# martenlienen/bsi

Hardware: AMD Instinct MI355X
Metric: images/sec BSI.sample k=128 (DiT, 3x32x32) (higher is better)
Workload: dtype bf16

## Files before the change

### bsi_amd/csrc/dit_ops.hip

```cpp
#include <math.h>

#include "common.h"
#include "dit_ops.h"

namespace {

constexpr int TPB = 256;

__global__ void silu_bf16_kernel(const float* __restrict__ pre, size_t n, __bf16* __restrict__ out) {
    for (size_t i = (size_t)blockIdx.x * blockDim.x + threadIdx.x; i < n; i += (size_t)gridDim.x * blockDim.x)
        out[i] = (__bf16)silu_f(pre[i]);
}

__global__ void cast_bf16_kernel(const float* __restrict__ in, int ld_in, int rows, int cols, __bf16* __restrict__ out, int ld) {
    const int r = blockIdx.y;
    const float* ir = in + (size_t)r * ld_in;
    __bf16* orow = out + (size_t)r * ld;
    for (int c = (blockIdx.x * blockDim.x + threadIdx.x) * 4; c < ld; c += gridDim.x * blockDim.x * 4) {
        float v[4];
#pragma unroll
        for (int k = 0; k < 4; ++k) v[k] = (c + k < cols) ? ir[c + k] : 0.0f;
        if (c + 3 < ld) {
            u32x2 w;
            w[0] = pack_bf16x2(v[0], v[1]);
            w[1] = pack_bf16x2(v[2], v[3]);
            *reinterpret_cast<u32x2*>(orow + c) = w;
        } else {
            for (int k = 0; k < 4 && c + k < ld; ++k) orow[c + k] = (__bf16)v[k];
        }
    }
}

__global__ void nyquist_kernel(const float* __restrict__ t, int rows, const float* __restrict__ scale,
                               const float* __restrict__ bias, int size, float* __restrict__ of, __bf16* __restrict__ ob) {
    const int r = blockIdx.y;
    const float tv = t[r];
    for (int j = blockIdx.x * blockDim.x + threadIdx.x; j < size; j += gridDim.x * blockDim.x) {
        const float v = sinf(__fmaf_rn(scale[j], tv, bias[j]));
        if (of) of[(size_t)r * size + j] = v;
        if (ob) ob[(size_t)r * size + j] = (__bf16)v;
    }
}

template <int VPL, bool MASKGEN = false>
__global__ void ln_modulate_kernel(float* __restrict__ x, int M, int d, float eps, const float* __restrict__ shift,
                                   const float* __restrict__ scale, int mod_rows, int mod_stride, int tokens,
                                   const float* __restrict__ ln_w, const float* __restrict__ ln_b,
                                   const __bf16* delta, const float* __restrict__ gate, __bf16* out, DropCfg dc,
                                   float* x_out, float* __restrict__ stats, const __bf16* delta0 = nullptr,
                                   const float* __restrict__ gate0 = nullptr, int write_x = 1, DropCfg mdc = DropCfg{},
                                   unsigned long long* __restrict__ maskw = nullptr) {
    const int lane = threadIdx.x & 63;
    const int row = blockIdx.x * (blockDim.x >> 6) + (threadIdx.x >> 6);
    if (row >= M) return;
    if constexpr (MASKGEN) maskw[(size_t)row * 64 + lane] = drop_mask_block(mdc, (unsigned)row, lane);
    const float* xr = x + (size_t)row * d;
    float* xw = (x_out ? x_out : x) + (size_t)row * d;
    const int d4 = d >> 2;
    const int mrow = (shift || gate || gate0) ? (row / tokens) % mod_rows : 0;
    f32x4 v[VPL];
    float s = 0.f;
#pragma unroll
    for (int i = 0; i < VPL; ++i) {
        const int c = i * 64 + lane;
        v[i] = (c < d4) ? reinterpret_cast<const f32x4*>(xr)[c] : f32x4{0.f, 0.f, 0.f, 0.f};
        if (delta0 && c < d4) {
            const u32x2 dw = __builtin_nontemporal_load(reinterpret_cast<const u32x2*>(delta0 + (size_t)row * d) + c);
            const f32x4 g = reinterpret_cast<const f32x4*>(gate0 + (size_t)mrow * mod_stride)[c];
            v[i][0] = __fmaf_rn(g[0], __uint_as_float(dw[0] << 16), v[i][0]);
            v[i][1] = __fmaf_rn(g[1], __uint_as_float(dw[0] & 0xffff0000u), v[i][1]);
            v[i][2] = __fmaf_rn(g[2], __uint_as_float(dw[1] << 16), v[i][2]);
            v[i][3] = __fmaf_rn(g[3], __uint_as_float(dw[1] & 0xffff0000u), v[i][3]);
        }
        if (delta && c < d4) {
            const u32x2 dw = __builtin_nontemporal_load(reinterpret_cast<const u32x2*>(delta + (size_t)row * d) + c);
            const f32x4 g = reinterpret_cast<const f32x4*>(gate + (size_t)mrow * mod_stride)[c];
            v[i][0] = __fmaf_rn(g[0], __uint_as_float(dw[0] << 16), v[i][0]);
            v[i][1] = __fmaf_rn(g[1], __uint_as_float(dw[0] & 0xffff0000u), v[i][1]);
            v[i][2] = __fmaf_rn(g[2], __uint_as_float(dw[1] << 16), v[i][2]);
            v[i][3] = __fmaf_rn(g[3], __uint_as_float(dw[1] & 0xffff0000u), v[i][3]);
            if (write_x) reinterpret_cast<f32x4*>(xw)[c] = v[i];
        }
        s += (v[i][0] + v[i][1]) + (v[i][2] + v[i][3]);
    }
    if (!out) return;
    const float mean = wave_sum(s) / (float)d;
    float q = 0.f;
#pragma unroll
    for (int i = 0; i < VPL; ++i) {
        const int c = i * 64 + lane;
        if (c < d4) {
#pragma unroll
            for (int k = 0; k < 4; ++k) {
                const float dd = v[i][k] - mean;
                q = __fmaf_rn(dd, dd, q);
            }
        }
    }
    const float rstd = 1.0f / sqrtf(wave_sum(q) / (float)d + eps);
    if (stats && lane == 0) {
        stats[2 * (size_t)row] = mean;
        stats[2 * (size_t)row + 1] = rstd;
    }
    const float* sh = shift ? shift + (size_t)mrow * mod_stride : nullptr;
    const float* sc = scale ? scale + (size_t)mrow * mod_stride : nullptr;
    __bf16* orow = out + (size_t)row * d;
#pragma unroll
    for (int i = 0; i < VPL; ++i) {
        const int c = i * 64 + lane;
        if (c < d4) {
            f32x4 y;
#pragma unroll
            for (int k = 0; k < 4; ++k) y[k] = (v[i][k] - mean) * rstd;
            if (sh) {
                const f32x4 a = reinterpret_cast<const f32x4*>(sh)[c];
                const f32x4 b = reinterpret_cast<const f32x4*>(sc)[c];
#pragma unroll
                for (int k = 0; k < 4; ++k) y[k] = __fmaf_rn(b[k] + 1.0f, y[k], a[k]);
            } else if (ln_w) {
                const f32x4 a = reinterpret_cast<const f32x4*>(ln_w)[c];
                const f32x4 b = reinterpret_cast<const f32x4*>(ln_b)[c];
#pragma unroll
                for (int k = 0; k < 4; ++k) y[k] = __fmaf_rn(y[k], a[k], b[k]);
            }
            if (dc.thr) {
                const unsigned rh = drop_row(dc, (unsigned)row);
#pragma unroll
                for (int k = 0; k < 4; ++k) y[k] = drop_keep_rc(dc, rh, (unsigned)c * 4 + k) ? y[k] * dc.scale : 0.0f;
            }
            u32x2 w;
            w[0] = pack_bf16x2(y[0], y[1]);
            w[1] = pack_bf16x2(y[2], y[3]);
            reinterpret_cast<u32x2*>(orow)[c] = w;
        }
    }
}

template <int VPL>
__global__ __launch_bounds__(256) void ln_modulate_stream_kernel(float* __restrict__ x, int M, int d, float eps, const float* __restrict__ shift,
                                                                 const float* __restrict__ scale, const __bf16* delta0,
                                                                 const float* __restrict__ gate0, const __bf16* delta,
                                                                 const float* __restrict__ gate, int write_x, __bf16* out) {
    __shared__ f32x4 tab[4][VPL * 64];
    const int d4 = d >> 2;
    for (int i = threadIdx.x; i < VPL * 64; i += blockDim.x) {
        const f32x4 z{0.f, 0.f, 0.f, 0.f};
        const bool in = i < d4;
        tab[0][i] = (gate0 && in) ? reinterpret_cast<const f32x4*>(gate0)[i] : z;
        tab[1][i] = (gate && in) ? reinterpret_cast<const f32x4*>(gate)[i] : z;
        tab[2][i] = in ? reinterpret_cast<const f32x4*>(shift)[i] : z;
        tab[3][i] = in ? reinterpret_cast<const f32x4*>(scale)[i] : z;
    }
    __syncthreads();
    const int lane = threadIdx.x & 63;
    const int wpb = blockDim.x >> 6;
    const int stride = gridDim.x * wpb;
    int row = blockIdx.x * wpb + (threadIdx.x >> 6);
    const bool has0 = delta0 != nullptr, has1 = delta != nullptr;

    struct Row {
        f32x4 v[VPL];
        u32x2 a[VPL], b[VPL];
    };
    auto load = [&](int r, Row& R) {
        const float* xr = x + (size_t)r * d;
#pragma unroll
        for (int i = 0; i < VPL; ++i) {
            const int c = i * 64 + lane;
            R.v[i] = (c < d4) ? reinterpret_cast<const f32x4*>(xr)[c] : f32x4{0.f, 0.f, 0.f, 0.f};
            if (has0 && c < d4) R.a[i] = __builtin_nontemporal_load(reinterpret_cast<const u32x2*>(delta0 + (size_t)r * d) + c);
            if (has1 && c < d4) R.b[i] = __builtin_nontemporal_load(reinterpret_cast<const u32x2*>(delta + (size_t)r * d) + c);
        }
    };
    auto finish = [&](int r, Row& R) {
        float* xw = x + (size_t)r * d;
        float s = 0.f;
#pragma unroll
        for (int i = 0; i < VPL; ++i) {
            const int c = i * 64 + lane;
            if (has0 && c < d4) {
                const f32x4 g = tab[0][c];
                R.v[i][0] = __fmaf_rn(g[0], __uint_as_float(R.a[i][0] << 16), R.v[i][0]);
                R.v[i][1] = __fmaf_rn(g[1], __uint_as_float(R.a[i][0] & 0xffff0000u), R.v[i][1]);
                R.v[i][2] = __fmaf_rn(g[2], __uint_as_float(R.a[i][1] << 16), R.v[i][2]);
                R.v[i][3] = __fmaf_rn(g[3], __uint_as_float(R.a[i][1] & 0xffff0000u), R.v[i][3]);
            }
            if (has1 && c < d4) {
                const f32x4 g = tab[1][c];
                R.v[i][0] = __fmaf_rn(g[0], __uint_as_float(R.b[i][0] << 16), R.v[i][0]);
                R.v[i][1] = __fmaf_rn(g[1], __uint_as_float(R.b[i][0] & 0xffff0000u), R.v[i][1]);
                R.v[i][2] = __fmaf_rn(g[2], __uint_as_float(R.b[i][1] << 16), R.v[i][2]);
                R.v[i][3] = __fmaf_rn(g[3], __uint_as_float(R.b[i][1] & 0xffff0000u), R.v[i][3]);
                if (write_x) reinterpret_cast<f32x4*>(xw)[c] = R.v[i];
            }
            s += (R.v[i][0] + R.v[i][1]) + (R.v[i][2] + R.v[i][3]);
        }
        const float mean = wave_sum(s) / (float)d;
        float q = 0.f;
#pragma unroll
        for (int i = 0; i < VPL; ++i) {
            const int c = i * 64 + lane;
            if (c < d4) {
#pragma unroll
                for (int k = 0; k < 4; ++k) {
                    const float dd = R.v[i][k] - mean;
                    q = __fmaf_rn(dd, dd, q);
                }
            }
        }
        const float rstd = 1.0f / sqrtf(wave_sum(q) / (float)d + eps);
        __bf16* orow = out + (size_t)r * d;
#pragma unroll
        for (int i = 0; i < VPL; ++i) {
            const int c = i * 64 + lane;
            if (c < d4) {
                f32x4 y;
#pragma unroll
                for (int k = 0; k < 4; ++k) y[k] = (R.v[i][k] - mean) * rstd;
                const f32x4 a = tab[2][c];
                const f32x4 b = tab[3][c];
#pragma unroll
                for (int k = 0; k < 4; ++k) y[k] = __fmaf_rn(b[k] + 1.0f, y[k], a[k]);
                u32x2 w;
                w[0] = pack_bf16x2(y[0], y[1]);
                w[1] = pack_bf16x2(y[2], y[3]);
                reinterpret_cast<u32x2*>(orow)[c] = w;
            }
        }
    };
    Row A, B;
    if (row >= M) return;
    load(row, A);
    while (true) {
        if (row + stride < M) load(row + stride, B);
        finish(row, A);
        row += stride;
        if (row >= M) break;
        if (row + stride < M) load(row + stride, A);
        finish(row, B);
        row += stride;
        if (row >= M) break;
    }
}

__global__ void fourier_features_kernel(const float* __restrict__ x, size_t total, int C, int inner, int nmin,
                                        int nfreq, float* __restrict__ out) {
    for (size_t idx = (size_t)blockIdx.x * blockDim.x + threadIdx.x; idx < total; idx += (size_t)gridDim.x * blockDim.x) {
        const size_t in_i = idx % inner;
        const size_t oc = idx / inner;
        const float v = x[idx];
        float* o = out + (oc * nfreq * 2) * inner + in_i;
        for (int n = 0; n < nfreq; ++n) {
            const float coef = 6.283185307179586f * (float)(1 << (nmin + n));
            o[(size_t)(n * 2 + 0) * inner] = sinf(__fmaf_rn(coef, v, 0.0f));
            o[(size_t)(n * 2 + 1) * inner] = sinf(__fmaf_rn(coef, v, 1.5707963267948966f));
        }
    }
}

__global__ void dit_prologue_kernel(const float* __restrict__ mu, const float* __restrict__ c_in, int coef_stride, int B,
                                    int C, int H, int W, int ps, int nmin, int nfreq, int kpad, __bf16* __restrict__ out) {
    const int HW = H * W;
    const size_t total = (size_t)B * HW;
    const int Cin = C + C * nfreq * 2;
    const int nw = W / ps;
    const int tokens = (H / ps) * nw;
    const int K = ps * ps * Cin;
    for (size_t idx = (size_t)blockIdx.x * blockDim.x + threadIdx.x; idx < total; idx += (size_t)gridDim.x * blockDim.x) {
        const int b = (int)(idx / HW);
        const int pix = (int)(idx % HW);
        const int h = pix / W, w = pix % W;
        const float ci = c_in ? c_in[(size_t)b * coef_stride] : 1.0f;
        const int tok = (h / ps) * nw + (w / ps);
        const int intra = (h % ps) * ps + (w % ps);
        __bf16* o = out + ((size_t)b * tokens + tok) * kpad + intra * Cin;
        for (int c = 0; c < C; ++c) {
            float v = mu[((size_t)b * C + c) * HW + pix];
            if (c_in) v = __fmul_rn(ci, v);
            o[c] = (__bf16)v;
            for (int n = 0; n < nfreq; ++n) {
                const float coef = 6.283185307179586f * (float)(1 << (nmin + n));
                o[C + (c * nfreq + n) * 2 + 0] = (__bf16)sinf(__fmaf_rn(coef, v, 0.0f));
                o[C + (c * nfreq + n) * 2 + 1] = (__bf16)sinf(__fmaf_rn(coef, v, 1.5707963267948966f));
            }
        }
        if (intra == ps * ps - 1) {
            __bf16* z = out + ((size_t)b * tokens + tok) * kpad;
            for (int c = K; c < kpad; ++c) z[c] = (__bf16)0.0f;
        }
    }
}

template <int VPL, bool WLDS>
__global__ void dit_final_kernel(const float* __restrict__ x, int Mtok, int d, int P, const float* __restrict__ ln_w,
                                 const float* __restrict__ ln_b, const float* __restrict__ dec_w,
                                 const float* __restrict__ dec_b, int C, int H, int W, int ps,
                                 const float* __restrict__ mu, const float* __restrict__ c_skip,
                                 const float* __restrict__ c_out, int coef_stride, const __bf16* __restrict__ delta,
                                 const float* __restrict__ gate, int gate_rows, int gate_stride,
                                 float* __restrict__ out) {
    extern __shared__ __attribute__((aligned(16))) float wsm[];
    const int d4 = d >> 2;
    if constexpr (WLDS) {
        for (int i = threadIdx.x; i < P * d4; i += blockDim.x)
            reinterpret_cast<f32x4*>(wsm)[i] = reinterpret_cast<const f32x4*>(dec_w)[i];
        __syncthreads();
    }
    const int lane = threadIdx.x & 63;
    const int wpb = blockDim.x >> 6;
    const int nw = W / ps;
    const int tokens = (H / ps) * nw;
    const int HW = H * W;
    constexpr int FR = 4;
    for (int row0 = (blockIdx.x * wpb + (threadIdx.x >> 6)) * FR; row0 < Mtok; row0 += gridDim.x * wpb * FR) {
        f32x4 v[FR][VPL];
        float s[FR], q[FR];
#pragma unroll
        for (int r = 0; r < FR; ++r) {
            const int row = row0 + r < Mtok ? row0 + r : Mtok - 1;
            const float* xr = x + (size_t)row * d;
            const int b_idx = row / tokens;
            s[r] = 0.f;
#pragma unroll
            for (int i = 0; i < VPL; ++i) {
                const int c = i * 64 + lane;
                v[r][i] = (c < d4) ? reinterpret_cast<const f32x4*>(xr)[c] : f32x4{0.f, 0.f, 0.f, 0.f};
                if (delta && c < d4) {
                    const u32x2 dw = reinterpret_cast<const u32x2*>(delta + (size_t)row * d)[c];
                    const f32x4 g = reinterpret_cast<const f32x4*>(gate + (size_t)(b_idx % gate_rows) * gate_stride)[c];
                    v[r][i][0] = __fmaf_rn(g[0], __uint_as_float(dw[0] << 16), v[r][i][0]);
                    v[r][i][1] = __fmaf_rn(g[1], __uint_as_float(dw[0] & 0xffff0000u), v[r][i][1]);
                    v[r][i][2] = __fmaf_rn(g[2], __uint_as_float(dw[1] << 16), v[r][i][2]);
                    v[r][i][3] = __fmaf_rn(g[3], __uint_as_float(dw[1] & 0xffff0000u), v[r][i][3]);
                }
                s[r] += (v[r][i][0] + v[r][i][1]) + (v[r][i][2] + v[r][i][3]);
            }
        }
#pragma unroll
        for (int m = 32; m > 0; m >>= 1)
#pragma unroll
            for (int r = 0; r < FR; ++r) s[r] += __shfl_xor(s[r], m, 64);
#pragma unroll
        for (int r = 0; r < FR; ++r) {
            const float mean = s[r] / (float)d;
            s[r] = mean;
            q[r] = 0.f;
#pragma unroll
            for (int i = 0; i < VPL; ++i) {
                const int c = i * 64 + lane;
                if (c < d4) {
#pragma unroll
                    for (int k = 0; k < 4; ++k) {
                        const float dd = v[r][i][k] - mean;
                        q[r] = __fmaf_rn(dd, dd, q[r]);
                    }
                }
            }
        }
#pragma unroll
        for (int m = 32; m > 0; m >>= 1)
#pragma unroll
            for (int r = 0; r < FR; ++r) q[r] += __shfl_xor(q[r], m, 64);
#pragma unroll
        for (int i = 0; i < VPL; ++i) {
            const int c = i * 64 + lane;
            if (c < d4) {
                const f32x4 a = reinterpret_cast<const f32x4*>(ln_w)[c];
                const f32x4 bb = reinterpret_cast<const f32x4*>(ln_b)[c];
#pragma unroll
                for (int r = 0; r < FR; ++r) {
                    const float rstd = 1.0f / sqrtf(q[r] / (float)d + 1e-5f);
#pragma unroll
                    for (int k = 0; k < 4; ++k) v[r][i][k] = __fmaf_rn((v[r][i][k] - s[r]) * rstd, a[k], bb[k]);
                }
            }
        }
        float mine[FR] = {0.f, 0.f, 0.f, 0.f};
        for (int o0 = 0; o0 < P; o0 += 4) {
            float acc[FR][4];
#pragma unroll
            for (int r = 0; r < FR; ++r)
#pragma unroll
                for (int u = 0; u < 4; ++u) acc[r][u] = 0.f;
#pragma unroll
            for (int u = 0; u < 4; ++u) {
                const int o = o0 + u < P ? o0 + u : P - 1;
#pragma unroll
                for (int i = 0; i < VPL; ++i) {
                    const int c = i * 64 + lane;
                    if (c < d4) {
                        const f32x4 wv = WLDS ? reinterpret_cast<const f32x4*>(wsm + (size_t)o * d)[c]
                                              : reinterpret_cast<const f32x4*>(dec_w + (size_t)o * d)[c];
#pragma unroll
                        for (int r = 0; r < FR; ++r)
#pragma unroll
                            for (int k = 0; k < 4; ++k) acc[r][u] = __fmaf_rn(v[r][i][k], wv[k], acc[r][u]);
                    }
                }
            }
#pragma unroll
            for (int m = 32; m > 0; m >>= 1)
#pragma unroll
                for (int r = 0; r < FR; ++r)
#pragma unroll
                    for (int u = 0; u < 4; ++u) acc[r][u] += __shfl_xor(acc[r][u], m, 64);
#pragma unroll
            for (int u = 0; u < 4; ++u)
                if (o0 + u < P && lane == o0 + u) {
#pragma unroll
                    for (int r = 0; r < FR; ++r) mine[r] = acc[r][u] + dec_b[o0 + u];
                }
        }
        if (lane < P) {
            const int intra = lane / C, ch = lane % C;
#pragma unroll
            for (int r = 0; r < FR; ++r) {
                const int row = row0 + r;
                if (row >= Mtok) break;
                const int b_idx = row / tokens, tok = row % tokens;
                const int th = tok / nw, tw = tok % nw;
                const int hh = th * ps + intra / ps, ww = tw * ps + intra % ps;
                const size_t gi = ((size_t)b_idx * C + ch) * HW + (size_t)hh * W + ww;
                float rr = mine[r];
                if (c_skip) {
                    const float cs = c_skip[(size_t)b_idx * coef_stride], co = c_out[(size_t)b_idx * coef_stride];
                    rr = __fmaf_rn(co, mine[r], __fmul_rn(cs, mu[gi]));
                }
                out[gi] = rr;
            }
        }
    }
}

}

#define S(stream) reinterpret_cast<hipStream_t>(stream)

extern "C" int bsi_cast_rows_bf16(const float* in, int ld_in, int rows, int cols, void* out, int ld_out,
                                  bsi_stream_t stream) {
    BSI_CHECK_ARG(in && out && rows > 0 && cols > 0 && ld_in >= cols && ld_out >= cols && ld_out % 4 == 0,
                  "bsi_cast_rows_bf16: bad args rows=%d cols=%d ld_in=%d ld_out=%d", rows, cols, ld_in, ld_out);
    int gx = (ld_out / 4 + TPB - 1) / TPB;
    if (gx > 16) gx = 16;
    hipLaunchKernelGGL(cast_bf16_kernel, dim3(gx, rows), dim3(TPB), 0, S(stream), in, ld_in, rows, cols,
                       reinterpret_cast<__bf16*>(out), ld_out);
    BSI_CHECK_LAUNCH("bsi_cast_bf16");
    return BSI_OK;
}

extern "C" int bsi_cast_bf16(const float* in, int rows, int cols, void* out, int ld_out, bsi_stream_t stream) {
    return bsi_cast_rows_bf16(in, cols, rows, cols, out, ld_out, stream);
}

extern "C" int bsi_silu_bf16(const float* pre, size_t n, void* out, bsi_stream_t stream) {
    BSI_CHECK_ARG(pre && out && n > 0, "bsi_silu_bf16: bad args");
    size_t g = (n + TPB - 1) / TPB;
    if (g > 4096) g = 4096;
    hipLaunchKernelGGL(silu_bf16_kernel, dim3((int)g), dim3(TPB), 0, S(stream), pre, n, reinterpret_cast<__bf16*>(out));
    BSI_CHECK_LAUNCH("bsi_silu_bf16");
    return BSI_OK;
}

extern "C" int bsi_fourier_features(const float* x, int outer, int C, int inner, int n_min, int n_max, float* out,
                                    bsi_stream_t stream) {
    BSI_CHECK_ARG(x && out && outer > 0 && C > 0 && inner > 0 && n_max >= n_min && n_min >= 0 && n_max < 31,
                  "bsi_fourier_features: bad args");
    const size_t total = (size_t)outer * C * inner;
    size_t g = (total + TPB - 1) / TPB;
    if (g > 8192) g = 8192;
    hipLaunchKernelGGL(fourier_features_kernel, dim3((int)g), dim3(TPB), 0, S(stream), x, total, C, inner, n_min,
                       n_max - n_min + 1, out);
    BSI_CHECK_LAUNCH("bsi_fourier_features");
    return BSI_OK;
}

extern "C" int bsi_nyquist_embed(const float* t, int rows, const float* scale, const float* bias, int size,
                                 float* out_f32, void* out_bf16, bsi_stream_t stream) {
    BSI_CHECK_ARG(t && scale && bias && rows > 0 && size > 0 && (out_f32 || out_bf16), "bsi_nyquist_embed: bad args");
    int gx = (size + TPB - 1) / TPB;
    hipLaunchKernelGGL(nyquist_kernel, dim3(gx, rows), dim3(TPB), 0, S(stream), t, rows, scale, bias, size, out_f32,
                       reinterpret_cast<__bf16*>(out_bf16));
    BSI_CHECK_LAUNCH("bsi_nyquist_embed");
    return BSI_OK;
}

int bsi_resid_ln_modulate_drop(float* x, int M, int d, float eps, const void* delta, const float* gate,
                               const float* shift, const float* scale, int mod_rows, int mod_stride, int tokens,
                               const float* ln_w, const float* ln_b, void* out_bf16, DropCfg dc, bsi_stream_t stream,
                               float* x_out, float* stats, const void* delta0, const float* gate0, int write_x, DropCfg mdc,
                               void* maskw) {
    BSI_CHECK_ARG(x && M > 0 && d > 0 && d % 4 == 0 && d <= 2048, "bsi_resid_ln_modulate: bad args M=%d d=%d", M, d);
    BSI_CHECK_ARG(out_bf16 || delta, "bsi_resid_ln_modulate: nothing to do");
    BSI_CHECK_ARG((shift == nullptr) == (scale == nullptr), "bsi_resid_ln_modulate: shift and scale go together");
    BSI_CHECK_ARG((delta == nullptr) == (gate == nullptr), "bsi_resid_ln_modulate: delta and gate go together");
    BSI_CHECK_ARG(!(shift || gate) || (mod_rows > 0 && tokens > 0 && mod_stride % 4 == 0),
                  "bsi_resid_ln_modulate: bad modulation table");
    BSI_CHECK_ARG((ln_w == nullptr) == (ln_b == nullptr), "bsi_resid_ln_modulate: ln weight and bias go together");
    BSI_CHECK_ARG((delta0 == nullptr) == (gate0 == nullptr) && (!delta0 || delta), "bsi_resid_ln_modulate: an older update needs its gate and a newer update");
    BSI_CHECK_ARG(write_x || (delta && out_bf16 && !x_out), "bsi_resid_ln_modulate: write_x = 0 needs an update and an output");
    BSI_CHECK_ARG(!(maskw && mdc.thr) || (d > 256 && d <= 1024 && out_bf16), "bsi_resid_ln_modulate: mask words ride on the d <= 1024 instance");
    const __bf16* dl0 = reinterpret_cast<const __bf16*>(delta0);
    const int wpb = TPB / 64;
    dim3 grid((M + wpb - 1) / wpb);
    __bf16* o = reinterpret_cast<__bf16*>(out_bf16);
    const __bf16* dl = reinterpret_cast<const __bf16*>(delta);
    if (g_bsi_ln_stream_cus > 0 && d > 256 && d <= 1024 && shift && o && mod_rows == 1 && !ln_w && !dc.thr && !x_out && !stats &&
        !(maskw && mdc.thr)) {
        static int per_cu = 0;
        if (per_cu == 0) {
            int n = 0;
            if (hipOccupancyMaxActiveBlocksPerMultiprocessor(&n, ln_modulate_stream_kernel<4>, TPB, 0) != hipSuccess || n < 1) n = 2;
            if (const char* e = getenv("BSI_LN_STREAM_WGS")) n = atoi(e) > 0 ? atoi(e) : n;
            per_cu = n;
        }
        int g = g_bsi_ln_stream_cus * per_cu;
        if (g > (int)grid.x) g = (int)grid.x;
        hipLaunchKernelGGL(ln_modulate_stream_kernel<4>, dim3(g), dim3(TPB), 0, S(stream), x, M, d, eps, shift, scale, dl0, gate0, dl,
                           gate, write_x, o);
        BSI_CHECK_LAUNCH("bsi_resid_ln_modulate");
        return BSI_OK;
    }
    if (d <= 256)
        hipLaunchKernelGGL(ln_modulate_kernel<1>, grid, dim3(TPB), 0, S(stream), x, M, d, eps, shift, scale, mod_rows,
                           mod_stride, tokens, ln_w, ln_b, dl, gate, o, dc, x_out, stats, dl0, gate0, write_x);
    else if (d <= 1024 && maskw && mdc.thr)
        hipLaunchKernelGGL((ln_modulate_kernel<4, true>), grid, dim3(TPB), 0, S(stream), x, M, d, eps, shift, scale, mod_rows,
                           mod_stride, tokens, ln_w, ln_b, dl, gate, o, dc, x_out, stats, dl0, gate0, write_x, mdc,
                           reinterpret_cast<unsigned long long*>(maskw));
    else if (d <= 1024)
        hipLaunchKernelGGL(ln_modulate_kernel<4>, grid, dim3(TPB), 0, S(stream), x, M, d, eps, shift, scale, mod_rows,
                           mod_stride, tokens, ln_w, ln_b, dl, gate, o, dc, x_out, stats, dl0, gate0, write_x);
    else
        hipLaunchKernelGGL(ln_modulate_kernel<8>, grid, dim3(TPB), 0, S(stream), x, M, d, eps, shift, scale, mod_rows,
                           mod_stride, tokens, ln_w, ln_b, dl, gate, o, dc, x_out, stats, dl0, gate0, write_x);
    BSI_CHECK_LAUNCH("bsi_resid_ln_modulate");
    return BSI_OK;
}

extern "C" int bsi_resid2_ln_modulate(float* x, int M, int d, float eps, const void* delta0, const float* gate0, const void* delta,
                                      const float* gate, int write_x, const float* shift, const float* scale, int mod_rows,
                                      int mod_stride, int tokens, void* out_bf16, bsi_stream_t stream) {
    return bsi_resid_ln_modulate_drop(x, M, d, eps, delta, gate, shift, scale, mod_rows, mod_stride, tokens, nullptr, nullptr,
                                      out_bf16, DropCfg{}, stream, nullptr, nullptr, delta0, gate0, write_x);
}

extern "C" int bsi_resid_ln_modulate(float* x, int M, int d, float eps, const void* delta, const float* gate,
                                     const float* shift, const float* scale, int mod_rows, int mod_stride, int tokens,
                                     const float* ln_w, const float* ln_b, void* out_bf16, bsi_stream_t stream) {
    return bsi_resid_ln_modulate_drop(x, M, d, eps, delta, gate, shift, scale, mod_rows, mod_stride, tokens, ln_w, ln_b,
                                      out_bf16, DropCfg{}, stream);
}

__global__ void dropout_mask_kernel(DropCfg dc, unsigned rows, unsigned cols, uint8_t* __restrict__ out) {
    const size_t n = (size_t)rows * cols;
    for (size_t i = (size_t)blockIdx.x * blockDim.x + threadIdx.x; i < n; i += (size_t)gridDim.x * blockDim.x) {
        const unsigned r = (unsigned)(i / cols), c = (unsigned)(i % cols);
        out[i] = drop_keep_rc(dc, drop_row(dc, r), c) ? 1 : 0;
    }
}

extern "C" int bsi_dropout_mask(float p, unsigned long long seed, unsigned site, unsigned rows, unsigned cols, uint8_t* out,
                                bsi_stream_t stream) {
    BSI_CHECK_ARG(out && rows > 0 && cols > 0 && p >= 0.f && p < 1.f, "bsi_dropout_mask: bad args");
    size_t g = ((size_t)rows * cols + TPB - 1) / TPB;
    if (g > 4096) g = 4096;
    hipLaunchKernelGGL(dropout_mask_kernel, dim3((int)g), dim3(TPB), 0, S(stream), make_drop(p, seed, site), rows, cols, out);
    BSI_CHECK_LAUNCH("bsi_dropout_mask");
    return BSI_OK;
}

extern "C" int bsi_ln_modulate(const float* x, int M, int d, float eps, const float* shift, const float* scale,
                               int mod_rows, int mod_stride, int tokens, const float* ln_w, const float* ln_b,
                               void* out_bf16, bsi_stream_t stream) {
    BSI_CHECK_ARG(out_bf16, "bsi_ln_modulate: null output");
    return bsi_resid_ln_modulate(const_cast<float*>(x), M, d, eps, nullptr, nullptr, shift, scale, mod_rows, mod_stride,
                                 tokens, ln_w, ln_b, out_bf16, stream);
}

int bsi_dit_prologue_launch(const float* mu, const float* c_in, int coef_stride, int B, int C, int H, int W, int ps,
                            int nmin, int nfreq, int kpad, void* out, hipStream_t s) {
    const size_t total = (size_t)B * H * W;
    size_t g = (total + TPB - 1) / TPB;
    if (g > 8192) g = 8192;
    hipLaunchKernelGGL(dit_prologue_kernel, dim3((int)g), dim3(TPB), 0, s, mu, c_in, coef_stride, B, C, H, W, ps, nmin,
                       nfreq, kpad, reinterpret_cast<__bf16*>(out));
    BSI_CHECK_LAUNCH("bsi_dit_prologue");
    return BSI_OK;
}

int bsi_dit_final_launch(const float* x, int Mtok, int d, int P, const float* ln_w, const float* ln_b,
                         const float* dec_w, const float* dec_b, int C, int H, int W, int ps, const float* mu,
                         const float* c_skip, const float* c_out, int coef_stride, const void* delta, const float* gate,
                         int gate_rows, int gate_stride, float* out, hipStream_t s) {
    size_t lds = (size_t)P * d * sizeof(float);
    if (P > 64) {
        bsi_set_error("bsi_dit_final: decoder P=%d unsupported (needs patch*patch*C <= 64)", P);
        return BSI_EINVAL;
    }
    const bool wlds = lds <= 128 * 1024;
    if (!wlds) lds = 0;
    const int wpb = TPB / 64;
    int grid = (Mtok + wpb * 4 - 1) / (wpb * 4);
    if (grid < 1) grid = 1;
    if (grid > 2048) grid = 2048;
#define LAUNCH_FINAL(V)                                                                                              \
    do {                                                                                                             \
        auto kern = wlds ? dit_final_kernel<V, true> : dit_final_kernel<V, false>;                                   \
        (void)hipFuncSetAttribute(reinterpret_cast<const void*>(kern), hipFuncAttributeMaxDynamicSharedMemorySize, (int)lds); \
        hipLaunchKernelGGL(kern, dim3(grid), dim3(TPB), lds, s, x, Mtok, d, P, ln_w, ln_b, dec_w, dec_b, C, H, W, ps, \
                           mu, c_skip, c_out, coef_stride, reinterpret_cast<const __bf16*>(delta), gate,             \
                           gate_rows > 0 ? gate_rows : 1, gate_stride, out);                                         \
    } while (0)
    if (d <= 256) LAUNCH_FINAL(1);
    else if (d <= 1024) LAUNCH_FINAL(4);
    else LAUNCH_FINAL(8);
#undef LAUNCH_FINAL
    BSI_CHECK_LAUNCH("bsi_dit_final");
    return BSI_OK;
}
```

Measured before the change: 49.10.

## Add two-rows-per-wave LN-modulate kernel and permlane/DPP wave reductions

```diff
diff --git a/bsi_amd/csrc/dit_ops.hip b/bsi_amd/csrc/dit_ops.hip
--- a/bsi_amd/csrc/dit_ops.hip
+++ b/bsi_amd/csrc/dit_ops.hip
@@ -40,6 +40,34 @@
         if (of) of[(size_t)r * size + j] = v;
         if (ob) ob[(size_t)r * size + j] = (__bf16)v;
     }
+}
+
+typedef unsigned u2v_ __attribute__((ext_vector_type(2)));
+__device__ __forceinline__ float fold32(float a, float b) {
+    const u2v_ t = __builtin_amdgcn_permlane32_swap(__float_as_uint(a), __float_as_uint(b), false, false);
+    return __uint_as_float(t[0]) + __uint_as_float(t[1]);
+}
+__device__ __forceinline__ float fold16(float a, float b) {
+    const u2v_ t = __builtin_amdgcn_permlane16_swap(__float_as_uint(a), __float_as_uint(b), false, false);
+    return __uint_as_float(t[0]) + __uint_as_float(t[1]);
+}
+__device__ __forceinline__ float row16_tree(float v) {
+    v = dpp_xadd<0x128>(v);
+    v = dpp_xadd<0x124>(v);
+    v = dpp_xadd<0x4E>(v);
+    return dpp_xadd<0xB1>(v);
+}
+__device__ __forceinline__ float lane_bcast(float v, int l) { return __int_as_float(__builtin_amdgcn_readlane(__float_as_int(v), l)); }
+__device__ __forceinline__ void wave_sum_x2(float& a, float& b) {
+    float t = fold32(a, b);
+    t = row16_tree(fold16(t, t));
+    a = lane_bcast(t, 0);
+    b = lane_bcast(t, 32);
+}
+__device__ __forceinline__ void wave_sum_x4(float (&s)[4]) {
+    const float t = row16_tree(fold16(fold32(s[0], s[2]), fold32(s[1], s[3])));
+#pragma unroll
+    for (int r = 0; r < 4; ++r) s[r] = lane_bcast(t, 16 * r);
 }
 
 template <int VPL, bool MASKGEN = false>
@@ -240,6 +268,102 @@
         finish(row, B);
         row += stride;
         if (row >= M) break;
+    }
+}
+
+constexpr int LN_RPW = 2;
+template <int VPL>
+__global__ __launch_bounds__(256) void ln_modulate_rows_kernel(float* x, int M, int d, float eps, const float* __restrict__ shift,
+                                                               const float* __restrict__ scale, const __bf16* delta0,
+                                                               const float* __restrict__ gate0, const __bf16* delta,
+                                                               const float* __restrict__ gate, int write_x, __bf16* out) {
+    constexpr int RPW = LN_RPW;
+    const int lane = threadIdx.x & 63;
+    const int row0 = (blockIdx.x * (blockDim.x >> 6) + (threadIdx.x >> 6)) * RPW;
+    if (row0 >= M) return;
+    const int d4 = d >> 2;
+    const bool has0 = delta0 != nullptr, has1 = delta != nullptr;
+    f32x4 v[RPW][VPL];
+    u32x2 a[RPW][VPL], b[RPW][VPL];
+#pragma unroll
+    for (int j = 0; j < RPW; ++j) {
+        const int r = row0 + j < M ? row0 + j : M - 1;
+#pragma unroll
+        for (int i = 0; i < VPL; ++i) {
+            const int c = i * 64 + lane;
+            v[j][i] = (c < d4) ? __builtin_nontemporal_load(reinterpret_cast<const f32x4*>(x + (size_t)r * d) + c) : f32x4{0.f, 0.f, 0.f, 0.f};
+            if (has0 && c < d4) a[j][i] = __builtin_nontemporal_load(reinterpret_cast<const u32x2*>(delta0 + (size_t)r * d) + c);
+            if (has1 && c < d4) b[j][i] = __builtin_nontemporal_load(reinterpret_cast<const u32x2*>(delta + (size_t)r * d) + c);
+        }
+    }
+    float s[RPW];
+#pragma unroll
+    for (int j = 0; j < RPW; ++j) s[j] = 0.f;
+#pragma unroll
+    for (int i = 0; i < VPL; ++i) {
+        const int c = i * 64 + lane;
+        if (has0 && c < d4) {
+            const f32x4 g = reinterpret_cast<const f32x4*>(gate0)[c];
+#pragma unroll
+            for (int j = 0; j < RPW; ++j) {
+                v[j][i][0] = __fmaf_rn(g[0], __uint_as_float(a[j][i][0] << 16), v[j][i][0]);
+                v[j][i][1] = __fmaf_rn(g[1], __uint_as_float(a[j][i][0] & 0xffff0000u), v[j][i][1]);
+                v[j][i][2] = __fmaf_rn(g[2], __uint_as_float(a[j][i][1] << 16), v[j][i][2]);
+                v[j][i][3] = __fmaf_rn(g[3], __uint_as_float(a[j][i][1] & 0xffff0000u), v[j][i][3]);
+            }
+        }
+        if (has1 && c < d4) {
+            const f32x4 g = reinterpret_cast<const f32x4*>(gate)[c];
+#pragma unroll
+            for (int j = 0; j < RPW; ++j) {
+                v[j][i][0] = __fmaf_rn(g[0], __uint_as_float(b[j][i][0] << 16), v[j][i][0]);
+                v[j][i][1] = __fmaf_rn(g[1], __uint_as_float(b[j][i][0] & 0xffff0000u), v[j][i][1]);
+                v[j][i][2] = __fmaf_rn(g[2], __uint_as_float(b[j][i][1] << 16), v[j][i][2]);
+                v[j][i][3] = __fmaf_rn(g[3], __uint_as_float(b[j][i][1] & 0xffff0000u), v[j][i][3]);
+                if (write_x && row0 + j < M) __builtin_nontemporal_store(v[j][i], reinterpret_cast<f32x4*>(x + (size_t)(row0 + j) * d) + c);
+            }
+        }
+#pragma unroll
+        for (int j = 0; j < RPW; ++j) s[j] += (v[j][i][0] + v[j][i][1]) + (v[j][i][2] + v[j][i][3]);
+    }
+    float q[RPW];
+    wave_sum_x2(s[0], s[1]);
+#pragma unroll
+    for (int j = 0; j < RPW; ++j) {
+        s[j] = s[j] / (float)d;
+        q[j] = 0.f;
+#pragma unroll
+        for (int i = 0; i < VPL; ++i) {
+            const int c = i * 64 + lane;
+            if (c < d4) {
+#pragma unroll
+                for (int k = 0; k < 4; ++k) {
+                    const float dd = v[j][i][k] - s[j];
+                    q[j] = __fmaf_rn(dd, dd, q[j]);
+                }
+            }
+        }
+    }
+    wave_sum_x2(q[0], q[1]);
+#pragma unroll
+    for (int j = 0; j < RPW; ++j) q[j] = 1.0f / sqrtf(q[j] / (float)d + eps);
+#pragma unroll
+    for (int i = 0; i < VPL; ++i) {
+        const int c = i * 64 + lane;
+        if (c < d4) {
+            const f32x4 sh = reinterpret_cast<const f32x4*>(shift)[c];
+            const f32x4 sc = reinterpret_cast<const f32x4*>(scale)[c];
+#pragma unroll
+            for (int j = 0; j < RPW; ++j) {
+                f32x4 y;
+#pragma unroll
+                for (int k = 0; k < 4; ++k) y[k] = __fmaf_rn(sc[k] + 1.0f, (v[j][i][k] - s[j]) * q[j], sh[k]);
+                u32x2 w;
+                w[0] = pack_bf16x2(y[0], y[1]);
+                w[1] = pack_bf16x2(y[2], y[3]);
+                if (row0 + j < M) reinterpret_cast<u32x2*>(out + (size_t)(row0 + j) * d)[c] = w;
+            }
+        }
     }
 }
 
@@ -324,9 +448,9 @@
 #pragma unroll
             for (int i = 0; i < VPL; ++i) {
                 const int c = i * 64 + lane;
-                v[r][i] = (c < d4) ? reinterpret_cast<const f32x4*>(xr)[c] : f32x4{0.f, 0.f, 0.f, 0.f};
+                v[r][i] = (c < d4) ? __builtin_nontemporal_load(reinterpret_cast<const f32x4*>(xr) + c) : f32x4{0.f, 0.f, 0.f, 0.f};
                 if (delta && c < d4) {
-                    const u32x2 dw = reinterpret_cast<const u32x2*>(delta + (size_t)row * d)[c];
+                    const u32x2 dw = __builtin_nontemporal_load(reinterpret_cast<const u32x2*>(delta + (size_t)row * d) + c);
                     const f32x4 g = reinterpret_cast<const f32x4*>(gate + (size_t)(b_idx % gate_rows) * gate_stride)[c];
                     v[r][i][0] = __fmaf_rn(g[0], __uint_as_float(dw[0] << 16), v[r][i][0]);
                     v[r][i][1] = __fmaf_rn(g[1], __uint_as_float(dw[0] & 0xffff0000u), v[r][i][1]);
@@ -336,10 +460,7 @@
                 s[r] += (v[r][i][0] + v[r][i][1]) + (v[r][i][2] + v[r][i][3]);
             }
         }
-#pragma unroll
-        for (int m = 32; m > 0; m >>= 1)
-#pragma unroll
-            for (int r = 0; r < FR; ++r) s[r] += __shfl_xor(s[r], m, 64);
+        wave_sum_x4(s);
 #pragma unroll
         for (int r = 0; r < FR; ++r) {
             const float mean = s[r] / (float)d;
@@ -357,10 +478,7 @@
                 }
             }
         }
-#pragma unroll
-        for (int m = 32; m > 0; m >>= 1)
-#pragma unroll
-            for (int r = 0; r < FR; ++r) q[r] += __shfl_xor(q[r], m, 64);
+        wave_sum_x4(q);
 #pragma unroll
         for (int i = 0; i < VPL; ++i) {
             const int c = i * 64 + lane;
@@ -375,56 +493,62 @@
                 }
             }
         }
-        float mine[FR] = {0.f, 0.f, 0.f, 0.f};
-        for (int o0 = 0; o0 < P; o0 += 4) {
-            float acc[FR][4];
-#pragma unroll
-            for (int r = 0; r < FR; ++r)
-#pragma unroll
-                for (int u = 0; u < 4; ++u) acc[r][u] = 0.f;
-#pragma unroll
-            for (int u = 0; u < 4; ++u) {
-                const int o = o0 + u < P ? o0 + u : P - 1;
-#pragma unroll
-                for (int i = 0; i < VPL; ++i) {
-                    const int c = i * 64 + lane;
-                    if (c < d4) {
-                        const f32x4 wv = WLDS ? reinterpret_cast<const f32x4*>(wsm + (size_t)o * d)[c]
-                                              : reinterpret_cast<const f32x4*>(dec_w + (size_t)o * d)[c];
-#pragma unroll
-                        for (int r = 0; r < FR; ++r)
-#pragma unroll
-                            for (int k = 0; k < 4; ++k) acc[r][u] = __fmaf_rn(v[r][i][k], wv[k], acc[r][u]);
+        const bool b3 = (lane & 8) != 0, b2 = (lane & 4) != 0;
+        for (int o0 = 0; o0 < P; o0 += 16) {
+            float mine = 0.f;
+#pragma unroll
+            for (int grp = 0; grp < 4; ++grp) {
+                const int ob = o0 + 4 * grp;
+                if (ob >= P) break;
+                float acc[FR][4];
+#pragma unroll
+                for (int r = 0; r < FR; ++r)
+#pragma unroll
+                    for (int u = 0; u < 4; ++u) acc[r][u] = 0.f;
+#pragma unroll
+                for (int u = 0; u < 4; ++u) {
+                    const int o = ob + u < P ? ob + u : P - 1;
+#pragma unroll
+                    for (int i = 0; i < VPL; ++i) {
+                        const int c = i * 64 + lane;
+                        if (c < d4) {
+                            const f32x4 wv = WLDS ? reinterpret_cast<const f32x4*>(wsm + (size_t)o * d)[c]
+                                                  : reinterpret_cast<const f32x4*>(dec_w + (size_t)o * d)[c];
+#pragma unroll
+                            for (int r = 0; r < FR; ++r)
+#pragma unroll
+                                for (int k = 0; k < 4; ++k) acc[r][u] = __fmaf_rn(v[r][i][k], wv[k], acc[r][u]);
+                        }
                     }
                 }
-            }
-#pragma unroll
-            for (int m = 32; m > 0; m >>= 1)
-#pragma unroll
-                for (int r = 0; r < FR; ++r)
-#pragma unroll
-                    for (int u = 0; u < 4; ++u) acc[r][u] += __shfl_xor(acc[r][u], m, 64);
-#pragma unroll
-            for (int u = 0; u < 4; ++u)
-                if (o0 + u < P && lane == o0 + u) {
-#pragma unroll
-                    for (int r = 0; r < FR; ++r) mine[r] = acc[r][u] + dec_b[o0 + u];
+                float a4[4];
+#pragma unroll
+                for (int u = 0; u < 4; ++u) a4[u] = fold16(fold32(acc[0][u], acc[2][u]), fold32(acc[1][u], acc[3][u]));
+                float a2[2];
+#pragma unroll
+                for (int u = 0; u < 2; ++u) {
+                    const float keep = b3 ? a4[u + 2] : a4[u], send = b3 ? a4[u] : a4[u + 2];
+                    a2[u] = keep + __int_as_float(__builtin_amdgcn_update_dpp(0, __float_as_int(send), 0x128, 0xf, 0xf, true));
                 }
-        }
-        if (lane < P) {
-            const int intra = lane / C, ch = lane % C;
-#pragma unroll
-            for (int r = 0; r < FR; ++r) {
-                const int row = row0 + r;
-                if (row >= Mtok) break;
+                const float keep = b2 ? a2[1] : a2[0], send = b2 ? a2[0] : a2[1];
+                float a1 = keep + __shfl_xor(send, 4, 64);
+                a1 = dpp_xadd<0x4E>(a1);
+                a1 = dpp_xadd<0xB1>(a1);
+                const int o = ob + ((lane >> 2) & 3);
+                if ((lane & 3) == grp && o < P) mine = a1 + dec_b[o];
+            }
+            const int o = o0 + 4 * (lane & 3) + ((lane >> 2) & 3);
+            const int row = row0 + (lane >> 4);
+            if (o < P && row < Mtok) {
+                const int intra = o / C, ch = o % C;
                 const int b_idx = row / tokens, tok = row % tokens;
                 const int th = tok / nw, tw = tok % nw;
                 const int hh = th * ps + intra / ps, ww = tw * ps + intra % ps;
                 const size_t gi = ((size_t)b_idx * C + ch) * HW + (size_t)hh * W + ww;
-                float rr = mine[r];
+                float rr = mine;
                 if (c_skip) {
                     const float cs = c_skip[(size_t)b_idx * coef_stride], co = c_out[(size_t)b_idx * coef_stride];
-                    rr = __fmaf_rn(co, mine[r], __fmul_rn(cs, mu[gi]));
+                    rr = __fmaf_rn(co, mine, __fmul_rn(cs, mu[gi]));
                 }
                 out[gi] = rr;
             }
@@ -520,6 +644,12 @@
         BSI_CHECK_LAUNCH("bsi_resid_ln_modulate");
         return BSI_OK;
     }
+    if (d > 256 && d <= 1024 && shift && o && mod_rows == 1 && !ln_w && !dc.thr && !x_out && !stats && !(maskw && mdc.thr)) {
+        hipLaunchKernelGGL(ln_modulate_rows_kernel<4>, dim3((M + wpb * LN_RPW - 1) / (wpb * LN_RPW)), dim3(TPB), 0, S(stream), x, M, d,
+                           eps, shift, scale, dl0, gate0, dl, gate, write_x, o);
+        BSI_CHECK_LAUNCH("bsi_resid_ln_modulate");
+        return BSI_OK;
+    }
     if (d <= 256)
         hipLaunchKernelGGL(ln_modulate_kernel<1>, grid, dim3(TPB), 0, S(stream), x, M, d, eps, shift, scale, mod_rows,
                            mod_stride, tokens, ln_w, ln_b, dl, gate, o, dc, x_out, stats, dl0, gate0, write_x);
```

Result: faster. 50.26 (median of 6 runs) (+2.4%).
